# zyt334/AdaFace

Measured on AMD Instinct MI355X. Metric: 512x512 images/sec @ 50 DDIM steps, batch 8, higher is better.
Workload: dtype bf16

## Files before the change

### adaface_amd/csrc/af_conv_gemm.hip

```cpp
#include "af_kernels.h"

#include <cstdlib>
#include <cstring>
#include <mutex>
#include <type_traits>

template <int BM, int BN> struct TileCfg {
  static constexpr int XR = BM / 32, WR = BN / 32;
  static constexpr int WM = BM / 2, WN = BN / 2;
  static constexpr int MI = WM / 32, NI = WN / 32;
  static constexpr int TILE_BYTES = (BM + BN) * 128;
  static constexpr int EPI_LD = BN + 4;
  static constexpr int EPI_BYTES = BM * EPI_LD * 4;
  static constexpr int LDS_BYTES = (2 * TILE_BYTES > EPI_BYTES) ? 2 * TILE_BYTES : EPI_BYTES;
};

__device__ __forceinline__ void lds_dma16(__amdgpu_buffer_rsrc_t rs, char* lds_base, unsigned voffset, unsigned soffset) {
#if defined(__HIP_DEVICE_COMPILE__)
  __builtin_amdgcn_raw_ptr_buffer_load_lds(rs, (__attribute__((address_space(3))) void*)lds_base, 16, voffset, soffset,
                                           0, 0);
#endif
}

__device__ __forceinline__ void tile_coords(int wg, int nwg, int ntm, int ntn, int gm, int& tm, int& tn) {
// ... 867 lines not shown
    char* base = smem + slot_off;
    pp_static_for<0, NPMAX>([&](auto qc) { stage_piece(qc, base, sc); });
    kw = kw_next(kw);
  };

  const unsigned lds0 = (unsigned)(__UINTPTR_TYPE__)((__attribute__((address_space(3))) char*)smem);
  const unsigned fch0 = (unsigned)((lane >> 4) ^ (lane & 7)) * 16u;
  const unsigned fch1 = (unsigned)(((lane >> 4) + 4) ^ (lane & 7)) * 16u;
  const unsigned x_base = (unsigned)((wq * 64 + (lane & 15)) * 128);
  const unsigned w_base = (unsigned)(XBYTES + (g * C::HN + (lane & 15)) * 128);

  f32x4 acc[NI][MI];
#pragma unroll
  for (int i = 0; i < NI; ++i)
#pragma unroll
    for (int j = 0; j < MI; ++j) acc[i][j] = f32x4{0.f, 0.f, 0.f, 0.f};
  pp_u32x4 xf[MI][2], wf[NI][2];
#pragma unroll
  for (int i = 0; i < NI; ++i) wf[i][1] = pp_u32x4{0u, 0u, 0u, 0u};
#pragma unroll
  for (int j = 0; j < MI; ++j) xf[j][1] = pp_u32x4{0u, 0u, 0u, 0u};

  auto half = [&](int slot_off, auto rc, auto mc) {
    constexpr int ur = decltype(rc)::value, um = decltype(mc)::value;
    const unsigned b = lds0 + (unsigned)slot_off + (ur ? fch1 : fch0);
    pp_static_for<0, NI * MI>([&](auto nc) {
      constexpr int n = decltype(nc)::value;
      constexpr int i = n / MI, j = n % MI;
      if constexpr (n < NI) wf[n][ur] = pp_lds_read128<n * 2048>(b + w_base);
      else if constexpr (n < NI + MI) xf[n - NI][ur] = pp_lds_read128<(n - NI) * 2048>(b + x_base);
      acc[i][j] = __builtin_amdgcn_mfma_f32_16x16x32_bf16(__builtin_bit_cast(bf16x8, wf[i][um]),
                                                          __builtin_bit_cast(bf16x8, xf[j][um]), acc[i][j], 0, 0, 0);
      if constexpr (n < NI + MI) __builtin_amdgcn_sched_barrier(0);
    });
  };
  std::integral_constant<int, 0> U0;
  std::integral_constant<int, 1> U1;

  const int cl = 4 * (lane >> 4);
  float4 bias_r[NI];
  auto load_bias = [&]() {
#pragma unroll
    for (int i = 0; i < NI; ++i) {
      bias_r[i] = float4{0.f, 0.f, 0.f, 0.f};
      if (p.bias && p.splitk <= 1) bias_r[i] = *reinterpret_cast<const float4*>(p.bias + n0 + g * C::HN + i * 16 + cl);
    }
  };
  if constexpr (!MG) load_bias();

  float4 ln_cs[LNMODE == 1 ? NI : 1];
  float ln_mu[LNMODE == 1 ? MI : 1], ln_rs[LNMODE == 1 ? MI : 1];
  if constexpr (LNMODE == 1) {
#pragma unroll
    for (int i = 0; i < NI; ++i) ln_cs[i] = *reinterpret_cast<const float4*>(p.ln_colsum + n0 + g * C::HN + i * 16 + cl);
#pragma unroll
    for (int j = 0; j < MI; ++j) {
      const int m = m0 + wq * 64 + j * 16 + (lane & 15);
      float2 st = float2{0.f, 0.f};
      if (m < p.M) st = *reinterpret_cast<const float2*>(p.ln_stats + (long)m * 2);
      ln_mu[j] = st.x;
      ln_rs[j] = st.y;
    }
  }

  pp_u32x4 w8[MG ? NI : 1][2], xa8[MG ? MI : 1][2], xb8[MG ? MI : 1][2];
  int wsc8[FP8 ? NI : 1];
  int xsc8 = p.x_scale_e8;
  if constexpr (MG && !FP8) {
#pragma unroll
    for (int i = 0; i < NI; ++i) w8[i][0] = w8[i][1] = pp_u32x4{0u, 0u, 0u, 0u};
#pragma unroll
    for (int j = 0; j < MI; ++j) xa8[j][0] = xa8[j][1] = xb8[j][0] = xb8[j][1] = pp_u32x4{0u, 0u, 0u, 0u};
  }
  if constexpr (FP8) {
    asm volatile("" : "+v"(xsc8));
#pragma unroll
    for (int i = 0; i < NI; ++i) {
      w8[i][0] = w8[i][1] = pp_u32x4{0u, 0u, 0u, 0u};
      wsc8[i] = (int)p.w_scale[n0 + g * C::HN + i * 16 + (lane & 15)];
    }
#pragma unroll
    for (int j = 0; j < MI; ++j) xa8[j][0] = xa8[j][1] = xb8[j][0] = xb8[j][1] = pp_u32x4{0u, 0u, 0u, 0u};
  }
  auto mfma8 = [&](f32x4& c, const pp_u32x4 (&wv)[2], const pp_u32x4 (&xv)[2], int wscale) {
    if constexpr (!FP8) {
      c = __builtin_amdgcn_mfma_f32_16x16x32_bf16(__builtin_bit_cast(bf16x8, wv[0]), __builtin_bit_cast(bf16x8, xv[0]), c, 0, 0, 0);
      c = __builtin_amdgcn_mfma_f32_16x16x32_bf16(__builtin_bit_cast(bf16x8, wv[1]), __builtin_bit_cast(bf16x8, xv[1]), c, 0, 0, 0);
      asm volatile("" : "+v"(c));
      return;
    }
    const pp_i32x8 a = __builtin_shufflevector(__builtin_bit_cast(pp_i32x4, wv[0]), __builtin_bit_cast(pp_i32x4, wv[1]), 0, 1, 2, 3, 4, 5, 6, 7);
    const pp_i32x8 b = __builtin_shufflevector(__builtin_bit_cast(pp_i32x4, xv[0]), __builtin_bit_cast(pp_i32x4, xv[1]), 0, 1, 2, 3, 4, 5, 6, 7);
    c = __builtin_amdgcn_mfma_scale_f32_16x16x128_f8f6f4(a, b, c, 0, 0, 0, wscale, 0, xsc8);
    asm volatile("" : "+v"(c));
  };
  auto wait_block = [&](auto nc, pp_u32x4 (&blk)[2]) {
    constexpr int n = decltype(nc)::value;
    asm volatile("s_waitcnt lgkmcnt(%2)" : "+v"(blk[0]), "+v"(blk[1]) : "n"(n) : "memory");
  };
#ifdef AF_LAB_ABLATE
  const int lab = p.ablate >> 4;
#else
  constexpr int lab = 0;
#endif
  auto cphase8 = [&](int slot_off, pp_u32x4 (&xc)[MG ? MI : 1][2], pp_u32x4 (&xp)[MG ? MI : 1][2], int stage_off,
                     const StageCtx& sc) {
    if constexpr (MG) {
      constexpr int NB = NI + MI;
      char* sbase = smem + stage_off;
      const unsigned b0 = lds0 + (unsigned)slot_off + fch0, b1 = lds0 + (unsigned)slot_off + fch1;
      auto rd_block = [&](auto bc) {
        constexpr int bi = decltype(bc)::value;
        if (lab & 2) return;
        if constexpr (bi == 0) {
          w8[0][0] = pp_lds_read128<0>(b0 + w_base);
          w8[0][1] = pp_lds_read128<0>(b1 + w_base);
        } else if constexpr (bi <= MI) {
          xc[bi - 1][0] = pp_lds_read128<(bi - 1) * 2048>(b0 + x_base);
          xc[bi - 1][1] = pp_lds_read128<(bi - 1) * 2048>(b1 + x_base);
        } else {
          w8[bi - MI][0] = pp_lds_read128<(bi - MI) * 2048>(b0 + w_base);
          w8[bi - MI][1] = pp_lds_read128<(bi - MI) * 2048>(b1 + w_base);
        }
      };
      rd_block(std::integral_constant<int, 0>{});
      rd_block(std::integral_constant<int, 1>{});
      __builtin_amdgcn_sched_barrier(0);
      pp_static_for<0, MI * NI>([&](auto mc) {
        constexpr int m = decltype(mc)::value;
        if constexpr (m < MI) {
          if (!(lab & 4)) mfma8(acc[NI - 1][m], w8[NI - 1], xp[m], wsc8[FP8 ? NI - 1 : 0]);
        } else {
          constexpr int i = (m - MI) / MI, j = (m - MI) % MI;
          constexpr int issued = (2 + m) < NB ? (2 + m) : NB;
          constexpr int need = i == 0 ? 1 + j : (j == 0 ? MI + i : -1);
          if constexpr (need >= 0) {
            std::integral_constant<int, 2 * (issued - need - 1)> cnt;
            if constexpr (i == 0) wait_block(cnt, xc[j]); else wait_block(cnt, w8[i]);
            if constexpr (i == 0 && j == 0) wait_block(cnt, w8[0]);
          }
          if (!(lab & 4)) mfma8(acc[i][j], w8[i], xc[j], wsc8[FP8 ? i : 0]);
        }
        if constexpr (2 + m < NB) rd_block(std::integral_constant<int, 2 + m>{});
        if constexpr (m >= MI && (m - MI) / 2 < NPMAX) {
          if (!(lab & 1) && g == ((m - MI) & 1)) stage_piece(std::integral_constant<int, (m - MI) / 2>{}, sbase, sc);
        }
        __builtin_amdgcn_sched_barrier(0);
      });
      static_assert(MI + 2 * (NPMAX - 1) + 1 < MI * NI, "merged schedule: a staging slot behind an MFMA for every piece");
      pp_wait_lgkm0();
    }
  };

  int rd = 0, w0 = SLOT, w1 = 2 * SLOT;
  if constexpr (MG) {
    stage(0);
    stage(SLOT);
    auto tile = [&](auto& xc, auto& xp) {
      if (g == 0) pp_wait_vm<NP0>(); else pp_wait_vm<NP1>();
      __builtin_amdgcn_s_barrier();
      const StageCtx sc = stage_begin(kw);
      cphase8(rd, xc, xp, w1, sc);
      kw = kw_next(kw);
      const int tmp = rd; rd = w0; w0 = w1; w1 = tmp;
    };
    for (int t = 0; t + 1 < KT; t += 2) {
      tile(xa8, xb8);
      tile(xb8, xa8);
    }
    if (KT & 1) tile(xa8, xb8);
    pp_wait_vm<0>();
    if (KT & 1) {
#pragma unroll
      for (int j = 0; j < MI; ++j) mfma8(acc[NI - 1][j], w8[NI - 1], xa8[j], wsc8[FP8 ? NI - 1 : 0]);
    } else {
#pragma unroll
      for (int j = 0; j < MI; ++j) mfma8(acc[NI - 1][j], w8[NI - 1], xb8[j], wsc8[FP8 ? NI - 1 : 0]);
    }
    __builtin_amdgcn_s_barrier();
  } else {
    auto wait_keep1 = [&]() { if (g == 0) pp_wait_vm<NP0>(); else pp_wait_vm<NP1>(); };
    stage(0);
    if (g == 1) {
      if (KT > 1) { stage(SLOT); wait_keep1(); } else pp_wait_vm<0>();
    }
    __builtin_amdgcn_s_barrier();
    if (g == 1) __builtin_amdgcn_s_barrier();
    auto dphase = [&](int t) {
      if (g == 0) {
        if (t + 1 < KT) { stage(w0); wait_keep1(); } else pp_wait_vm<0>();
      } else {
        if (t + 2 < KT) stage(w1);
      }
      __builtin_amdgcn_s_barrier();
    };
    auto cend = [&](int t) {
      if (g == 1) { if (t + 2 < KT) wait_keep1(); else pp_wait_vm<0>(); }
      __builtin_amdgcn_s_barrier();
      const int tmp = rd; rd = w0; w0 = w1; w1 = tmp;
    };
    for (int t = 0; t < KT; ++t) {
      dphase(t);
      __builtin_amdgcn_s_setprio(1);
      half(rd, U0, U1);
      pp_wait_lgkm0();
      half(rd, U1, U0);
      pp_wait_lgkm0();
      __builtin_amdgcn_s_setprio(0);
      cend(t);
    }
#pragma unroll
    for (int i = 0; i < NI; ++i)
#pragma unroll
      for (int j = 0; j < MI; ++j)
        acc[i][j] = __builtin_amdgcn_mfma_f32_16x16x32_bf16(__builtin_bit_cast(bf16x8, wf[i][1]),
                                                            __builtin_bit_cast(bf16x8, xf[j][1]), acc[i][j], 0, 0, 0);
    if (g == 0) __builtin_amdgcn_s_barrier();
  }
  if constexpr (MG) load_bias();

  pp_epilogue<BN, LNMODE>(p, acc, bias_r, ln_cs, ln_mu, ln_rs, smem, tid, lane, g, wq, m0, n0, tn, zk);
}

#ifdef AF_LAB_ABLATE
__device__ unsigned long long g_lab_stamps[2048 * 5];
extern "C" int af_lab_stamps(unsigned long long* out, int n) {
  return hipMemcpyFromSymbol(out, HIP_SYMBOL(g_lab_stamps), sizeof(unsigned long long) * (size_t)n) == hipSuccess ? 0 : -1;
}
__device__ __forceinline__ unsigned long long lab_now() {
  unsigned long long t;
  __builtin_amdgcn_sched_barrier(0);
  asm volatile("s_memrealtime %0\n\ts_waitcnt lgkmcnt(0)" : "=s"(t)::"memory");
  __builtin_amdgcn_sched_barrier(0);
  return t;
}
#endif
struct Halo8Cfg {
  static constexpr int BN = 160;
  static constexpr int HPIX = 400, HBUF = HPIX * 128, WBYTES = BN * 128;
  static constexpr int W_BASE = 2 * HBUF, LDS_BYTES = 2 * HBUF + 3 * WBYTES;
  static constexpr int NHQ = 7;
  static_assert(LDS_BYTES <= 160 * 1024, "LDS budget");
};

template <int LABL>
__global__ __launch_bounds__(512) void conv3x3_halo8_kernel(const ConvGemmParams p) {
  using C = PpCfg<160>;
  using H = Halo8Cfg;
  typedef bf16 T;
  constexpr int BN = 160, NI = C::NI, MI = C::MI, NHQ = H::NHQ;
  extern __shared__ __attribute__((aligned(1024))) char smem[];
  const int tid = threadIdx.x, lane = tid & 63, wid = __builtin_amdgcn_readfirstlane(tid >> 6);
  const int g = wid >> 2, wq = wid & 3;
  const int ntm = p.M / 256, ntn = p.N / BN;
  int tm, tn;
  tile_coords(blockIdx.x, gridDim.x, ntm, ntn, p.group_m, tm, tn);
  const int m0 = tm * 256, n0 = tn * BN;
  const int zk = blockIdx.z;
  T* const xsrc = const_cast<T*>(reinterpret_cast<const T*>(p.src));
  T* const wsrc = const_cast<T*>(reinterpret_cast<const T*>(p.W));
  const __amdgpu_buffer_rsrc_t rs_x = __builtin_amdgcn_make_buffer_rsrc(xsrc, 0, (int)0xFFFFFFF0u, 0x00020000);
  const __amdgpu_buffer_rsrc_t rs_w = __builtin_amdgcn_make_buffer_rsrc(wsrc, 0, (int)0xFFFFFFF0u, 0x00020000);

  const int KT_all = p.K / 64;
  const int kt_per = (KT_all + p.splitk - 1) / p.splitk;
  const int kt_begin = zk * kt_per;
#ifdef AF_LAB_ABLATE
  const int lab = p.ablate >> 4;
  const int KT = (lab & 16) ? 9 : min(KT_all, kt_begin + kt_per) - kt_begin;
#else
  constexpr int lab = 0;
  const int KT = min(KT_all, kt_begin + kt_per) - kt_begin;
#endif
  const int chunk0 = kt_begin / 9;
  const int nch = KT / 9;
#ifdef AF_LAB_ABLATE
  unsigned long long st0 = 0, st1 = 0, st2 = 0;
  if (lab & 64) st0 = lab_now();
#endif

  const int Wo = p.Wo, HW = Wo + 2, wsh = p.wo_shift;
  const int R = 256 >> wsh;
  const int HP = (R + 2) * HW;
  const int img = m0 >> p.howo_shift;
  const int y0 = (m0 & (p.Ho * Wo - 1)) >> wsh;
  const int srow = lane >> 3;
  const unsigned dchunk = (unsigned)((lane & 7) ^ srow);
  const unsigned ldcb = (unsigned)p.ldc * 2u;

  unsigned h_off[NHQ];
  const int nhq = (H::HPIX / 8 - 1 - wid) / 8 + 1;
#pragma unroll
  for (int q = 0; q < NHQ; ++q) {
    const int hp = (wid + 8 * q) * 8 + srow;
    const int hy = hp / HW, hx = hp - hy * HW;
    const int iy = y0 - 1 + hy, ix = hx - 1;
    const bool ok = hp < HP && (unsigned)iy < (unsigned)p.Hi && (unsigned)ix < (unsigned)p.Wi;
    h_off[q] = ok ? (unsigned)((long)img * p.src_batch_stride * 2) + (unsigned)((iy >> p.up) * p.Ws + (ix >> p.up)) * ldcb + dchunk * 16u
                  : 0xFFFFFFFFu;
  }
  const unsigned hl6 = (unsigned)(wid < 2 ? 8 * (NHQ - 1) * 1024 : 0);
  if (wid >= 2) h_off[NHQ - 1] = h_off[0];
  unsigned w_off[3];
#pragma unroll
  for (int q = 0; q < 3; ++q) {
    const int n = n0 + (wid + 8 * q) * 8 + srow;
    w_off[q] = (n < p.Wrows && (wid + 8 * q) < BN / 8) ? (unsigned)((long)n * p.ldw * 2) + dchunk * 16u : 0xFFFFFFFFu;
  }
// ... 1714 lines not shown
```

### adaface_amd/csrc/af_conv_s8.hip

```cpp
#include "af_kernels.h"

#include <type_traits>

namespace cs8 {
typedef bf16 T;
typedef __attribute__((ext_vector_type(4))) unsigned u32x4;
constexpr int BM = 256, BN = 80, NI = 5, MI = 2, SPLITK = 4;
constexpr int HSLOTS = 448, HBUF = HSLOTS * 128, NHQ = HSLOTS / 8 / 8;
constexpr int WBYTES = BN * 128, WPIECES = BN / 8, D = 3, NS = 4;
constexpr int W_BASE = 2 * HBUF, LDS_BYTES = W_BASE + NS * WBYTES;
static_assert(LDS_BYTES <= 160 * 1024 && NHQ == 7, "LDS plan");

__device__ __forceinline__ void lds_dma16(__amdgpu_buffer_rsrc_t rs, char* lds_base, unsigned voffset, unsigned soffset) {
#if defined(__HIP_DEVICE_COMPILE__)
  __builtin_amdgcn_raw_ptr_buffer_load_lds(rs, (__attribute__((address_space(3))) void*)lds_base, 16, voffset, soffset, 0, 0);
#endif
}
__device__ __forceinline__ u32x4 lds_read128(unsigned addr) {
  u32x4 v;
  asm volatile("ds_read_b128 %0, %1" : "=v"(v) : "v"(addr) : "memory");
  return v;
}
template <int OFF> __device__ __forceinline__ u32x4 lds_read128o(unsigned addr) {
  u32x4 v;
  asm volatile("ds_read_b128 %0, %1 offset:%2" : "=v"(v) : "v"(addr), "n"(OFF) : "memory");
  return v;
}
template <int N> __device__ __forceinline__ void wait_vm() { asm volatile("s_waitcnt vmcnt(%0)" ::"n"(N) : "memory"); }
template <int N> __device__ __forceinline__ void wait_lgkm2(u32x4& a, u32x4& b) {
  asm volatile("s_waitcnt lgkmcnt(%2)" : "+v"(a), "+v"(b) : "n"(N) : "memory");
}
template <int N> __device__ __forceinline__ void wait_lgkm4(u32x4& a, u32x4& b, u32x4& c, u32x4& d) {
  asm volatile("s_waitcnt lgkmcnt(%4)" : "+v"(a), "+v"(b), "+v"(c), "+v"(d) : "n"(N) : "memory");
}
template <int I, int N, typename F> __device__ __forceinline__ void static_for(F&& f) {
  if constexpr (I < N) {
    f(std::integral_constant<int, I>{});
    static_for<I + 1, N>(f);
  }
}
__device__ __forceinline__ f32x4 mma(const u32x4& a, const u32x4& b, const f32x4& c) {
  return __builtin_amdgcn_mfma_f32_16x16x32_bf16(__builtin_bit_cast(bf16x8, a), __builtin_bit_cast(bf16x8, b), c, 0, 0, 0);
}

template <int SPLITK_T>
__global__ __launch_bounds__(512) void conv3x3_s8_kernel(const ConvGemmParams p) {
  extern __shared__ __attribute__((aligned(1024))) char smem[];
  const int tid = threadIdx.x, lane = tid & 63, wid = __builtin_amdgcn_readfirstlane(tid >> 6);
  const int l15 = lane & 15, g = lane >> 4;
  const int ntn = p.N / BN;
  const int tm = blockIdx.x / ntn, tn = blockIdx.x - tm * ntn;
  const int m0 = tm * BM, n0 = tn * BN, zk = blockIdx.z;
  const int nch = (p.Cin >> 6) / SPLITK_T, chunk0 = zk * nch;
  const __amdgpu_buffer_rsrc_t rs_x = __builtin_amdgcn_make_buffer_rsrc(const_cast<T*>(reinterpret_cast<const T*>(p.src)), 0, (int)0xFFFFFFF0u, 0x00020000);
  const __amdgpu_buffer_rsrc_t rs_w = __builtin_amdgcn_make_buffer_rsrc(const_cast<T*>(reinterpret_cast<const T*>(p.W)), 0, (int)0xFFFFFFF0u, 0x00020000);

  const int srow = lane >> 3;
  const unsigned dchunk = (unsigned)((lane & 7) ^ srow);
  const unsigned ldcb = (unsigned)p.ldc * 2u;
  const int wsh = p.wo_shift, Wo = 1 << wsh, HW = Wo + 2, hwsh = p.howo_shift;
  const int R = min(p.Ho, 256 >> wsh), HP1 = (R + 2) * HW, ipt = 256 / (R << wsh);
  const int img0 = m0 >> hwsh, y0 = (m0 & ((1 << hwsh) - 1)) >> wsh;
  unsigned h_off[NHQ];
#pragma unroll
  for (int q = 0; q < NHQ; ++q) {
    const int hp = (wid + 8 * q) * 8 + srow;
    const int img = hp / HP1, rem = hp - img * HP1, hy = rem / HW, hx = rem - hy * HW;
    const int iy = y0 + hy - 1, ix = hx - 1;
    const bool ok = img < ipt && (unsigned)iy < (unsigned)p.Ho && (unsigned)ix < (unsigned)Wo;
    h_off[q] = ok ? (unsigned)(((img0 + img) << hwsh) + (iy << wsh) + ix) * ldcb + dchunk * 16u : 0xFFFFFFFFu;
  }
  const int nwq = wid < WPIECES - 8 ? 2 : 1;
  unsigned w_off[2];
#pragma unroll
  for (int q = 0; q < 2; ++q) w_off[q] = (unsigned)((n0 + (wid + 8 * q) * 8 + srow) * p.ldw * 2) + dchunk * 16u;

  const int nsteps = nch * 9;
  auto stage_w = [&](int s, int slot) {
    const int c = s / 9, tap = s - 9 * c;
    const bool live = s < nsteps;
    const unsigned k0b = (unsigned)(tap * p.Cin + (chunk0 + c) * 64) * 2u;
    lds_dma16(rs_w, smem + W_BASE + slot * WBYTES + wid * 1024, live ? w_off[0] : 0xFFFFFFFFu, k0b);
    if (wid < WPIECES - 8) lds_dma16(rs_w, smem + W_BASE + slot * WBYTES + (wid + 8) * 1024, live ? w_off[1] : 0xFFFFFFFFu, k0b);
  };
  auto stage_h = [&](auto qc, int hbuf, int c) {
    constexpr int q = decltype(qc)::value;
    const bool live = c < nch;
    lds_dma16(rs_x, smem + hbuf * HBUF + (wid + 8 * q) * 1024, live ? h_off[q] : 0xFFFFFFFFu, (unsigned)(chunk0 + c) * 128u);
  };

  const unsigned lds0 = (unsigned)(__UINTPTR_TYPE__)((__attribute__((address_space(3))) char*)smem);
  const unsigned fch0 = (unsigned)(g ^ (lane & 7)) * 16u, fch1 = (unsigned)((g + 4) ^ (lane & 7)) * 16u;
  const unsigned w_base = (unsigned)(l15 * 128);
  int xhp[MI];
#pragma unroll
  for (int j = 0; j < MI; ++j) {
    const int t = wid * 32 + j * 16 + l15;
    const int part = t / (R << wsh), yl = (t >> wsh) - part * R;
    xhp[j] = part * HP1 + yl * HW + (t & (Wo - 1));
  }
  f32x4 acc[NI][MI];
#pragma unroll
  for (int i = 0; i < NI; ++i)
#pragma unroll
    for (int j = 0; j < MI; ++j) acc[i][j] = f32x4{0.f, 0.f, 0.f, 0.f};

  static_for<0, NHQ>([&](auto qc) { stage_h(qc, 0, 0); });
#pragma unroll
  for (int s = 0; s < D; ++s) stage_w(s, s);

  u32x4 xs[2][MI][2], wh[2][2][2];
#pragma unroll
  for (int j = 0; j < MI; ++j) xs[1][j][0] = xs[1][j][1] = u32x4{0u, 0u, 0u, 0u};
#pragma unroll
  for (int b2 = 0; b2 < 2; ++b2) wh[1][b2][0] = wh[1][b2][1] = u32x4{0u, 0u, 0u, 0u};
  int hb = 0, slot = 0;
  for (int c = 0; c < nch; ++c) {
    static_for<0, 9>([&](auto tc) {
      constexpr int tap = decltype(tc)::value;
      constexpr int cs = tap & 1, ps = cs ^ 1;
      constexpr int hyoung = tap == 0 ? 0 : (tap == 1 ? 1 : (tap == 2 ? 2 : (tap <= 7 ? 3 : 2)));
      if (nwq == 2) wait_vm<2 * (D - 1) + hyoung>(); else wait_vm<(D - 1) + hyoung>();
      __builtin_amdgcn_s_barrier();
      constexpr int ky = tap / 3, kx = tap - 3 * ky;
      const int tapoff = ky * HW + kx;
      unsigned xa[MI];
#pragma unroll
      for (int j = 0; j < MI; ++j) {
        const unsigned hp = (unsigned)(xhp[j] + tapoff);
        xa[j] = lds0 + (unsigned)(hb * HBUF) + (hp << 7) + ((((unsigned)g ^ hp) & 7u) << 4);
      }
      const unsigned wa0 = lds0 + (unsigned)(W_BASE + slot * WBYTES) + w_base + fch0;
      const unsigned wa1 = lds0 + (unsigned)(W_BASE + slot * WBYTES) + w_base + fch1;
      u32x4 wf[3][2];
#pragma unroll
      for (int j = 0; j < MI; ++j) {
        xs[cs][j][0] = lds_read128(xa[j]);
        xs[cs][j][1] = lds_read128(xa[j] ^ 64u);
      }
      wf[0][0] = lds_read128o<0 * 2048>(wa0); wf[0][1] = lds_read128o<0 * 2048>(wa1);
      wf[1][0] = lds_read128o<1 * 2048>(wa0); wf[1][1] = lds_read128o<1 * 2048>(wa1);
      wf[2][0] = lds_read128o<2 * 2048>(wa0); wf[2][1] = lds_read128o<2 * 2048>(wa1);
      __builtin_amdgcn_sched_barrier(0);
#pragma unroll
      for (int b2 = 0; b2 < 2; ++b2)
#pragma unroll
        for (int j = 0; j < MI; ++j) {
          acc[3 + b2][j] = mma(wh[ps][b2][0], xs[ps][j][0], acc[3 + b2][j]);
          acc[3 + b2][j] = mma(wh[ps][b2][1], xs[ps][j][1], acc[3 + b2][j]);
          asm volatile("" : "+v"(acc[3 + b2][j]));
        }
      __builtin_amdgcn_sched_barrier(0);
      wait_lgkm4<4>(xs[cs][0][0], xs[cs][0][1], xs[cs][1][0], xs[cs][1][1]);
      wait_lgkm2<4>(wf[0][0], wf[0][1]);
#pragma unroll
      for (int j = 0; j < MI; ++j) {
        acc[0][j] = mma(wf[0][0], xs[cs][j][0], acc[0][j]);
        acc[0][j] = mma(wf[0][1], xs[cs][j][1], acc[0][j]);
        asm volatile("" : "+v"(acc[0][j]));
      }
      wh[cs][0][0] = lds_read128o<3 * 2048>(wa0); wh[cs][0][1] = lds_read128o<3 * 2048>(wa1);
      __builtin_amdgcn_sched_barrier(0);
      wait_lgkm2<4>(wf[1][0], wf[1][1]);
#pragma unroll
      for (int j = 0; j < MI; ++j) {
        acc[1][j] = mma(wf[1][0], xs[cs][j][0], acc[1][j]);
        acc[1][j] = mma(wf[1][1], xs[cs][j][1], acc[1][j]);
        asm volatile("" : "+v"(acc[1][j]));
      }
      stage_w(c * 9 + tap + D, (slot + D) & (NS - 1));
      if constexpr (tap < NHQ) stage_h(std::integral_constant<int, tap>{}, hb ^ 1, c + 1);
      wh[cs][1][0] = lds_read128o<4 * 2048>(wa0); wh[cs][1][1] = lds_read128o<4 * 2048>(wa1);
      __builtin_amdgcn_sched_barrier(0);
      wait_lgkm2<4>(wf[2][0], wf[2][1]);
#pragma unroll
      for (int j = 0; j < MI; ++j) {
        acc[2][j] = mma(wf[2][0], xs[cs][j][0], acc[2][j]);
        acc[2][j] = mma(wf[2][1], xs[cs][j][1], acc[2][j]);
        asm volatile("" : "+v"(acc[2][j]));
      }
      __builtin_amdgcn_sched_barrier(0);
      asm volatile("s_waitcnt lgkmcnt(0)"
                   : "+v"(wh[cs][0][0]), "+v"(wh[cs][0][1]), "+v"(wh[cs][1][0]), "+v"(wh[cs][1][1])
                   :
                   : "memory");
      slot = (slot + 1) & (NS - 1);
    });
#pragma unroll
    for (int j = 0; j < MI; ++j) { xs[1][j][0] = xs[0][j][0]; xs[1][j][1] = xs[0][j][1]; }
#pragma unroll
    for (int b2 = 0; b2 < 2; ++b2) { wh[1][b2][0] = wh[0][b2][0]; wh[1][b2][1] = wh[0][b2][1]; }
    hb ^= 1;
  }
#pragma unroll
  for (int b2 = 0; b2 < 2; ++b2)
#pragma unroll
    for (int j = 0; j < MI; ++j) {
      acc[3 + b2][j] = mma(wh[1][b2][0], xs[1][j][0], acc[3 + b2][j]);
      acc[3 + b2][j] = mma(wh[1][b2][1], xs[1][j][1], acc[3 + b2][j]);
    }
  wait_vm<0>();

  if constexpr (SPLITK_T > 1) {
    float* slab = reinterpret_cast<float*>(p.ws) + (long)zk * p.M * p.N;
#pragma unroll
    for (int j = 0; j < MI; ++j) {
      const int m = m0 + wid * 32 + j * 16 + l15;
#pragma unroll
      for (int i = 0; i < NI; ++i) *reinterpret_cast<f32x4*>(slab + (long)m * p.N + n0 + i * 16 + 4 * g) = acc[i][j];
    }
  } else {
    __builtin_amdgcn_s_barrier();
    constexpr int OPITCH = BN * 2 + 16, OCH = BN / 8, NST = 32 * OCH / 64;
    char* otile = smem + wid * (32 * OPITCH);
    const T* res = reinterpret_cast<const T*>(p.residual);
    const T* rowb = reinterpret_cast<const T*>(p.rowbias);
    const int cl = 4 * g;
    float4 bvec[NI];
    Quad<T> bq[NI];
#pragma unroll
    for (int i = 0; i < NI; ++i) {
      bvec[i] = p.bias ? *reinterpret_cast<const float4*>(p.bias + n0 + i * 16 + cl) : float4{0.f, 0.f, 0.f, 0.f};
      if (rowb) bq[i].load(rowb + (long)(m0 >> p.howo_shift) * p.ldrb + n0 + i * 16 + cl);
    }
#pragma unroll
    for (int j = 0; j < MI; ++j) {
      const int m = m0 + wid * 32 + j * 16 + l15;
      Quad<T> rq[NI];
      if (res) {
#pragma unroll
        for (int i = 0; i < NI; ++i) rq[i].load(res + (long)m * p.ldr + n0 + i * 16 + cl);
      }
#pragma unroll
      for (int i = 0; i < NI; ++i) {
        const float* bp = reinterpret_cast<const float*>(&bvec[i]);
        Quad<T> o;
#pragma unroll
        for (int e = 0; e < 4; ++e) {
          float v = acc[i][j][e] + bp[e];
          if (rowb) v += to_f32<T>(bq[i].e[e]);
          if (res) v += to_f32<T>(rq[i].e[e]);
          o.e[e] = from_f32<T>(v);
        }
        o.store(reinterpret_cast<T*>(otile + (j * 16 + l15) * OPITCH) + i * 16 + cl);
      }
    }
    const __amdgpu_buffer_rsrc_t rs_o = __builtin_amdgcn_make_buffer_rsrc(reinterpret_cast<T*>(p.out), 0, (int)0xFFFFFFF0u, 0x00020000);
    u32x4 chunk[NST];
    unsigned orow[NST];
#pragma unroll
    for (int i = 0; i < NST; ++i) {
      const unsigned c = (unsigned)(lane + 64 * i), row = c / OCH, ch = c - row * OCH;
      orow[i] = (unsigned)(m0 + wid * 32 + (int)row) * (unsigned)(p.ldo * 2) + ch * 16u;
      chunk[i] = *reinterpret_cast<const u32x4*>(otile + row * OPITCH + ch * 16);
    }
    __builtin_amdgcn_sched_barrier(0);
#pragma unroll
    for (int i = 0; i < NST; ++i) __builtin_amdgcn_raw_buffer_store_b128(chunk[i], rs_o, orow[i], n0 * 2, 0);
    __builtin_amdgcn_sched_barrier(0);
  }
}
}

int af_conv_s8_slices(const ConvGemmParams& p, int batch) {
  auto pow2 = [](int v) { return v > 0 && (v & (v - 1)) == 0; };
  if (batch != 1 || p.fp8 || p.ks != 3 || p.stride != 1 || p.pad != 1 || p.up != 0 || p.Hi != p.Ho || p.Wi != p.Wo ||
      p.Hs != p.Ho || p.Ws != p.Wo || !pow2(p.Wo) || !pow2(p.Ho) || p.Wo < 8 || p.Wo > 64 || p.M <= 0 || p.M % cs8::BM != 0 || p.N % cs8::BN != 0 ||
      p.K != 9 * p.Cin || p.ldc < p.Cin || p.ldc % 8 != 0 || p.epilogue != AF_EPI_NONE || p.ln_stats || p.ln_stats_out || p.gn_ab || p.phase4 ||
      p.src_batch_stride != (long)p.Ho * p.Wo * p.ldc)
    return 0;
  const int R = p.Ho < 256 / p.Wo ? p.Ho : 256 / p.Wo;
  if (256 % (R * p.Wo) != 0 || (256 / (R * p.Wo)) * (R + 2) * (p.Wo + 2) > cs8::HSLOTS || (p.Ho * p.Wo > 256 && p.Ho % R != 0)) return 0;
  if (p.Wo == 8 && p.Ho == 8) return p.Cin % (64 * cs8::SPLITK) == 0 ? cs8::SPLITK : 0;
  return (p.Cin % 64 == 0 && p.ldo % 8 == 0 && (!p.residual || p.ldr % 4 == 0) && (!p.rowbias || p.ldrb % 4 == 0) && ((__UINTPTR_TYPE__)p.out & 15) == 0 &&
          (long)(p.M / cs8::BM) * (p.N / cs8::BN) >= 128) ? 1 : 0;
}
bool af_conv_s8_ok(const ConvGemmParams& p, int batch) { return af_conv_s8_slices(p, batch) != 0; }
int af_launch_conv_s8(const ConvGemmParams& p, hipStream_t stream) {
  static unsigned long long attr_done4 = 0, attr_done1 = 0;
  const int sl = af_conv_s8_slices(p, 1);
  if (sl == 0 || p.splitk != sl || (sl > 1 && !p.ws) || p.wo_shift < 3 || p.howo_shift < p.wo_shift) {
    af_set_error_msg("conv_s8: shape / slice count %d not taken by the small-map kernel", p.splitk);
    return -1;
  }
  const dim3 grid((p.M / cs8::BM) * (p.N / cs8::BN), 1, sl);
  if (sl > 1) {
    if (int rc = af_ensure_dynamic_lds(attr_done4, reinterpret_cast<const void*>(&cs8::conv3x3_s8_kernel<cs8::SPLITK>), cs8::LDS_BYTES)) return rc;
    hipLaunchKernelGGL(cs8::conv3x3_s8_kernel<cs8::SPLITK>, grid, dim3(512), cs8::LDS_BYTES, stream, p);
  } else {
    if (int rc = af_ensure_dynamic_lds(attr_done1, reinterpret_cast<const void*>(&cs8::conv3x3_s8_kernel<1>), cs8::LDS_BYTES)) return rc;
    hipLaunchKernelGGL(cs8::conv3x3_s8_kernel<1>, grid, dim3(512), cs8::LDS_BYTES, stream, p);
  }
  HIP_CHECK_RET(hipGetLastError());
  return 0;
}
```

Before: 10.99.

## Specialize bf16 merged-group GEMM main loop with compile-time slot rotation and incremental walk

Adds a dedicated main-loop path for the non-FP8 merged-group case. The loop is unrolled six steps deep so the triple-buffer LDS slot offsets and register ping-pong choices become compile-time constants. The runtime index swaps and per-tile stage_begin/kw_next recomputation are replaced by an incremental walk struct that carries channel, tap and offset state forward. The group branch (g) is hoisted out of the loop. This should cut scalar address arithmetic and branching per K-tile, at the cost of larger code size and more register pressure.

```diff
diff --git a/adaface_amd/csrc/af_conv_gemm.hip b/adaface_amd/csrc/af_conv_gemm.hip
--- a/adaface_amd/csrc/af_conv_gemm.hip
+++ b/adaface_amd/csrc/af_conv_gemm.hip
@@ -1043,8 +1043,176 @@
     }
   };
 
+  struct PpWalk {
+    int kt, tap, kx;
+    unsigned c0b, k0b;
+    unsigned delta;
+  };
+  struct PpStage {
+    __amdgpu_buffer_rsrc_t rx, rw;
+    unsigned c0b, k0b, delta;
+    int tapbit;
+  };
+  const int kt_end = kt_begin + KT;
+  const unsigned cin2 = (unsigned)p.Cin * 2u, rowstep = (unsigned)(p.Ws - p.ks + 1) * ldcb;
+  auto walk_next = [&](PpWalk w) -> PpWalk {
+    ++w.kt;
+    if constexpr (GATHER) {
+      const bool row = w.kx + 1 == p.ks, chunk = w.tap + 1 == taps8;
+      w.kx = row ? 0 : w.kx + 1;
+      w.delta = chunk ? 0u : w.delta + (row ? rowstep : ldcb);
+      w.c0b += chunk ? 128u : 0u;
+      w.k0b = chunk ? w.c0b : w.k0b + cin2;
+      w.tap = chunk ? 0 : w.tap + 1;
+    } else {
+      w.c0b += 128u;
+      w.k0b = w.c0b;
+    }
+    return w;
+  };
+  auto stage_vals = [&](const PpWalk& w) -> PpStage {
+    PpStage s;
+    const int nrec = w.kt < kt_end ? (int)0xFFFFFFF0u : 0;
+    s.rx = __builtin_amdgcn_make_buffer_rsrc(const_cast<T*>(reinterpret_cast<const T*>(p.src)), 0, nrec, 0x00020000);
+    s.rw = __builtin_amdgcn_make_buffer_rsrc(const_cast<T*>(reinterpret_cast<const T*>(p.W)), 0, nrec, 0x00020000);
+    s.c0b = w.c0b;
+    s.k0b = w.k0b;
+    s.delta = w.delta;
+    s.tapbit = 1 << w.tap;
+#ifdef AF_LAB_ABLATE
+    if ((p.ablate & 0x100) && w.tap) s.tapbit = 0;
+#endif
+    return s;
+  };
+  auto piece16 = [&](auto qc, auto gc, char* base, const PpStage& s) {
+    constexpr int q = decltype(qc)::value, G = decltype(gc)::value;
+    constexpr int NX = G ? NX1 : NX0, NP = G ? NP1 : NP0, XB = G ? XP0 : 0, WB = G ? WP0 : 0;
+    if constexpr (q < NX) {
+      unsigned a = x_off[q];
+      if constexpr (GATHER) a = (x_yx[q] & s.tapbit) ? a + s.delta : 0xFFFFFFFFu;
+      lds_dma16(s.rx, base + (XB + wq + 4 * q) * 1024, a, s.c0b);
+    } else if constexpr (q < NP) {
+      lds_dma16(s.rw, base + XBYTES + (WB + wq + 4 * (q - NX)) * 1024, w_off[q - NX], s.k0b);
+    }
+  };
+  auto step16 = [&](auto sc, auto gc, PpWalk w) -> PpWalk {
+    constexpr int S = decltype(sc)::value, G = decltype(gc)::value;
+    constexpr int NB = NI + MI, RD = (S % 3) * SLOT, ST = ((S + 2) % 3) * SLOT;
+    auto& xc = (S & 1) ? xb8 : xa8;
+    auto& xp = (S & 1) ? xa8 : xb8;
+    pp_wait_vm<G ? NP1 : NP0>();
+    __builtin_amdgcn_s_barrier();
+    const PpStage s = stage_vals(w);
+    const unsigned b0 = lds0 + (unsigned)RD + fch0, b1 = lds0 + (unsigned)RD + fch1;
+    auto rd_block = [&](auto bc) {
+      constexpr int bi = decltype(bc)::value;
+      if (lab & 2) return;
+      if constexpr (bi == 0) {
+        w8[0][0] = pp_lds_read128<0>(b0 + w_base);
+        w8[0][1] = pp_lds_read128<0>(b1 + w_base);
+      } else if constexpr (bi <= MI) {
+        xc[bi - 1][0] = pp_lds_read128<(bi - 1) * 2048>(b0 + x_base);
+        xc[bi - 1][1] = pp_lds_read128<(bi - 1) * 2048>(b1 + x_base);
+      } else {
+        w8[bi - MI][0] = pp_lds_read128<(bi - MI) * 2048>(b0 + w_base);
+        w8[bi - MI][1] = pp_lds_read128<(bi - MI) * 2048>(b1 + w_base);
+      }
+    };
+    rd_block(std::integral_constant<int, 0>{});
+    rd_block(std::integral_constant<int, 1>{});
+    __builtin_amdgcn_sched_barrier(0);
+    pp_static_for<0, MI * NI>([&](auto mc) {
+      constexpr int m = decltype(mc)::value;
+      if constexpr (m < MI) {
+        if (!(lab & 4)) mfma8(acc[NI - 1][m], w8[NI - 1], xp[m], 0);
+      } else {
+        constexpr int i = (m - MI) / MI, j = (m - MI) % MI;
+        constexpr int issued = (2 + m) < NB ? (2 + m) : NB;
+        constexpr int need = i == 0 ? 1 + j : (j == 0 ? MI + i : -1);
+        if constexpr (need >= 0) {
+          std::integral_constant<int, 2 * (issued - need - 1)> cnt;
+          if constexpr (i == 0) wait_block(cnt, xc[j]); else wait_block(cnt, w8[i]);
+          if constexpr (i == 0 && j == 0) wait_block(cnt, w8[0]);
+        }
+        if (!(lab & 4)) mfma8(acc[i][j], w8[i], xc[j], 0);
+      }
+      if constexpr (2 + m < NB) rd_block(std::integral_constant<int, 2 + m>{});
+      if constexpr (m >= MI && ((m - MI) & 1) == G && (m - MI) / 2 < NPMAX) {
+        if (!(lab & 1)) piece16(std::integral_constant<int, (m - MI) / 2>{}, gc, smem + ST, s);
+      }
+      __builtin_amdgcn_sched_barrier(0);
+    });
+    pp_wait_lgkm0();
+    return walk_next(w);
+  };
+  auto run16 = [&](auto gc, PpWalk w) {
+    std::integral_constant<int, 0> S0; std::integral_constant<int, 1> S1; std::integral_constant<int, 2> S2;
+    std::integral_constant<int, 3> S3; std::integral_constant<int, 4> S4; std::integral_constant<int, 5> S5;
+    for (int n = KT / 6; n > 0; --n) {
+      w = step16(S0, gc, w);
+      w = step16(S1, gc, w);
+      w = step16(S2, gc, w);
+      w = step16(S3, gc, w);
+      w = step16(S4, gc, w);
+      w = step16(S5, gc, w);
+    }
+    const int r = KT % 6;
+    if (r > 0) {
+      w = step16(S0, gc, w);
+      if (r > 1) {
+        w = step16(S1, gc, w);
+        if (r > 2) {
+          w = step16(S2, gc, w);
+          if (r > 3) {
+            w = step16(S3, gc, w);
+            if (r > 4) step16(S4, gc, w);
+          }
+        }
+      }
+    }
+  };
+
   int rd = 0, w0 = SLOT, w1 = 2 * SLOT;
-  if constexpr (MG) {
+  if constexpr (MG && !FP8) {
+    PpWalk w;
+    {
+      const int cc = kt_begin / taps8, tap = kt_begin - cc * taps8, ky = tap / p.ks;
+      w.kt = kt_begin;
+      w.tap = tap;
+      w.kx = tap - ky * p.ks;
+      w.c0b = (unsigned)cc * 128u;
+      w.k0b = (unsigned)(tap * p.Cin + cc * 64) * 2u;
+      w.delta = (unsigned)(ky * p.Ws + w.kx) * ldcb;
+    }
+    std::integral_constant<int, 0> G0;
+    std::integral_constant<int, 1> G1;
+    auto stage16 = [&](auto gc, auto slc, const PpWalk& k) {
+      const PpStage s = stage_vals(k);
+      pp_static_for<0, NPMAX>([&](auto qc) { piece16(qc, gc, smem + decltype(slc)::value * SLOT, s); });
+    };
+    std::integral_constant<int, 0> L0;
+    std::integral_constant<int, 1> L1;
+    if (g == 0) {
+      stage16(G0, L0, w);
+      w = walk_next(w);
+      stage16(G0, L1, w);
+      run16(G0, walk_next(w));
+    } else {
+      stage16(G1, L0, w);
+      w = walk_next(w);
+      stage16(G1, L1, w);
+      run16(G1, walk_next(w));
+    }
+    pp_wait_vm<0>();
+    if (KT & 1) {
+#pragma unroll
+      for (int j = 0; j < MI; ++j) mfma8(acc[NI - 1][j], w8[NI - 1], xa8[j], 0);
+    } else {
+#pragma unroll
+      for (int j = 0; j < MI; ++j) mfma8(acc[NI - 1][j], w8[NI - 1], xb8[j], 0);
+    }
+    __builtin_amdgcn_s_barrier();
+  } else if constexpr (MG) {
     stage(0);
     stage(SLOT);
     auto tile = [&](auto& xc, auto& xp) {
```

Result: no change. 11.02 (median of 6 runs) (+0.3%).

## Restage small-map conv pipeline per kernel row with interleaved LDS prefetch

Applied to the files above, without the earlier changes.

Reworks the 3x3 small-map conv main loop so weights are staged one kernel row (three taps) at a time into two double-buffered slots, and the halo buffer shrinks to 50 pieces. LDS reads for the next tap are interleaved with the MFMA blocks of the current tap, with fine-grained lgkmcnt waits. Global-memory waits and barriers now happen only once per kernel row instead of every tap. It also adds compile-time ablation variants behind AF_LAB_ABLATE that can skip DMA, LDS reads or MFMAs for lab experiments. The risk is the hand-tuned waitcnt counts: if any is wrong the kernel reads stale data, and the extra in-flight reads can raise register pressure.

```diff
diff --git a/adaface_amd/csrc/af_conv_s8.hip b/adaface_amd/csrc/af_conv_s8.hip
--- a/adaface_amd/csrc/af_conv_s8.hip
+++ b/adaface_amd/csrc/af_conv_s8.hip
@@ -6,24 +6,20 @@
 typedef bf16 T;
 typedef __attribute__((ext_vector_type(4))) unsigned u32x4;
 constexpr int BM = 256, BN = 80, NI = 5, MI = 2, SPLITK = 4;
-constexpr int HSLOTS = 448, HBUF = HSLOTS * 128, NHQ = HSLOTS / 8 / 8;
-constexpr int WBYTES = BN * 128, WPIECES = BN / 8, D = 3, NS = 4;
-constexpr int W_BASE = 2 * HBUF, LDS_BYTES = W_BASE + NS * WBYTES;
-static_assert(LDS_BYTES <= 160 * 1024 && NHQ == 7, "LDS plan");
+constexpr int HPIECES = 50, HSLOTS = HPIECES * 8, HBUF = HSLOTS * 128, NHQ = 7;
+constexpr int WBYTES = BN * 128, WPIECES = BN / 8, WSLOT = 3 * WBYTES;
+constexpr int W_BASE = 2 * HBUF, LDS_BYTES = W_BASE + 2 * WSLOT;
+static_assert(LDS_BYTES <= 160 * 1024 && (NHQ - 1) * 8 < HPIECES && NHQ * 8 >= HPIECES && HPIECES - 48 == WPIECES - 8, "LDS plan");
 
 __device__ __forceinline__ void lds_dma16(__amdgpu_buffer_rsrc_t rs, char* lds_base, unsigned voffset, unsigned soffset) {
 #if defined(__HIP_DEVICE_COMPILE__)
   __builtin_amdgcn_raw_ptr_buffer_load_lds(rs, (__attribute__((address_space(3))) void*)lds_base, 16, voffset, soffset, 0, 0);
 #endif
 }
-__device__ __forceinline__ u32x4 lds_read128(unsigned addr) {
+template <int LABL, int OFF> __device__ __forceinline__ u32x4 lds_read128o(unsigned addr) {
   u32x4 v;
-  asm volatile("ds_read_b128 %0, %1" : "=v"(v) : "v"(addr) : "memory");
-  return v;
-}
-template <int OFF> __device__ __forceinline__ u32x4 lds_read128o(unsigned addr) {
-  u32x4 v;
-  asm volatile("ds_read_b128 %0, %1 offset:%2" : "=v"(v) : "v"(addr), "n"(OFF) : "memory");
+  if constexpr ((LABL & 2) != 0) asm volatile("" : "=v"(v) : "v"(addr) : "memory");
+  else asm volatile("ds_read_b128 %0, %1 offset:%2" : "=v"(v) : "v"(addr), "n"(OFF) : "memory");
   return v;
 }
 template <int N> __device__ __forceinline__ void wait_vm() { asm volatile("s_waitcnt vmcnt(%0)" ::"n"(N) : "memory"); }
@@ -39,12 +35,17 @@
     static_for<I + 1, N>(f);
   }
 }
-__device__ __forceinline__ f32x4 mma(const u32x4& a, const u32x4& b, const f32x4& c) {
-  return __builtin_amdgcn_mfma_f32_16x16x32_bf16(__builtin_bit_cast(bf16x8, a), __builtin_bit_cast(bf16x8, b), c, 0, 0, 0);
-}
-
-template <int SPLITK_T>
-__global__ __launch_bounds__(512) void conv3x3_s8_kernel(const ConvGemmParams p) {
+template <int LABL> __device__ __forceinline__ f32x4 mma(const u32x4& a, const u32x4& b, const f32x4& c) {
+  if constexpr ((LABL & 4) != 0) {
+    f32x4 d = c;
+    asm volatile("" : "+v"(d) : "v"(a), "v"(b));
+    return d;
+  } else {
+    return __builtin_amdgcn_mfma_f32_16x16x32_bf16(__builtin_bit_cast(bf16x8, a), __builtin_bit_cast(bf16x8, b), c, 0, 0, 0);
+  }
+}
+
+template <int SPLITK_T, int LABL> __device__ __forceinline__ void conv3x3_s8_body(const ConvGemmParams& p) {
   extern __shared__ __attribute__((aligned(1024))) char smem[];
   const int tid = threadIdx.x, lane = tid & 63, wid = __builtin_amdgcn_readfirstlane(tid >> 6);
   const int l15 = lane & 15, g = lane >> 4;
@@ -70,18 +71,23 @@
     const bool ok = img < ipt && (unsigned)iy < (unsigned)p.Ho && (unsigned)ix < (unsigned)Wo;
     h_off[q] = ok ? (unsigned)(((img0 + img) << hwsh) + (iy << wsh) + ix) * ldcb + dchunk * 16u : 0xFFFFFFFFu;
   }
-  const int nwq = wid < WPIECES - 8 ? 2 : 1;
+  const bool two = wid < WPIECES - 8;
   unsigned w_off[2];
 #pragma unroll
   for (int q = 0; q < 2; ++q) w_off[q] = (unsigned)((n0 + (wid + 8 * q) * 8 + srow) * p.ldw * 2) + dchunk * 16u;
 
-  const int nsteps = nch * 9;
-  auto stage_w = [&](int s, int slot) {
-    const int c = s / 9, tap = s - 9 * c;
-    const bool live = s < nsteps;
-    const unsigned k0b = (unsigned)(tap * p.Cin + (chunk0 + c) * 64) * 2u;
-    lds_dma16(rs_w, smem + W_BASE + slot * WBYTES + wid * 1024, live ? w_off[0] : 0xFFFFFFFFu, k0b);
-    if (wid < WPIECES - 8) lds_dma16(rs_w, smem + W_BASE + slot * WBYTES + (wid + 8) * 1024, live ? w_off[1] : 0xFFFFFFFFu, k0b);
+  auto stage_w = [&](auto kxc, auto qc, int c, int ky, int slot) {
+    constexpr int kx = decltype(kxc)::value, q = decltype(qc)::value;
+    const bool live = c < nch;
+    const unsigned k0b = (unsigned)((3 * ky + kx) * p.Cin + (chunk0 + c) * 64) * 2u;
+    lds_dma16(rs_w, smem + W_BASE + slot * WSLOT + kx * WBYTES + (wid + 8 * q) * 1024, live ? w_off[q] : 0xFFFFFFFFu, k0b);
+  };
+  auto stage_step_w = [&](auto kxc, int c, int ky, int slot) {
+    constexpr int kx = decltype(kxc)::value;
+    stage_w(kxc, std::integral_constant<int, 0>{}, c, ky, slot);
+    if constexpr (kx == 2) {
+      if (two) static_for<0, 3>([&](auto k2) { stage_w(k2, std::integral_constant<int, 1>{}, c, ky, slot); });
+    }
   };
   auto stage_h = [&](auto qc, int hbuf, int c) {
     constexpr int q = decltype(qc)::value;
@@ -105,99 +111,100 @@
 #pragma unroll
     for (int j = 0; j < MI; ++j) acc[i][j] = f32x4{0.f, 0.f, 0.f, 0.f};
 
-  static_for<0, NHQ>([&](auto qc) { stage_h(qc, 0, 0); });
-#pragma unroll
-  for (int s = 0; s < D; ++s) stage_w(s, s);
-
-  u32x4 xs[2][MI][2], wh[2][2][2];
+  static_for<0, NHQ - 1>([&](auto qc) { stage_h(qc, 0, 0); });
+  if (two) stage_h(std::integral_constant<int, NHQ - 1>{}, 0, 0);
+  static_for<0, 3>([&](auto kxc) { stage_step_w(kxc, 0, 0, 0); });
+
+  u32x4 xs[2][MI][2], wf[2][NI][2];
 #pragma unroll
   for (int j = 0; j < MI; ++j) xs[1][j][0] = xs[1][j][1] = u32x4{0u, 0u, 0u, 0u};
 #pragma unroll
-  for (int b2 = 0; b2 < 2; ++b2) wh[1][b2][0] = wh[1][b2][1] = u32x4{0u, 0u, 0u, 0u};
+  for (int b = 3; b < NI; ++b) wf[1][b][0] = wf[1][b][1] = u32x4{0u, 0u, 0u, 0u};
   int hb = 0, slot = 0;
+  if constexpr ((LABL & 8) == 0)
   for (int c = 0; c < nch; ++c) {
     static_for<0, 9>([&](auto tc) {
       constexpr int tap = decltype(tc)::value;
-      constexpr int cs = tap & 1, ps = cs ^ 1;
-      constexpr int hyoung = tap == 0 ? 0 : (tap == 1 ? 1 : (tap == 2 ? 2 : (tap <= 7 ? 3 : 2)));
-      if (nwq == 2) wait_vm<2 * (D - 1) + hyoung>(); else wait_vm<(D - 1) + hyoung>();
-      __builtin_amdgcn_s_barrier();
-      constexpr int ky = tap / 3, kx = tap - 3 * ky;
-      const int tapoff = ky * HW + kx;
-      unsigned xa[MI];
-#pragma unroll
-      for (int j = 0; j < MI; ++j) {
-        const unsigned hp = (unsigned)(xhp[j] + tapoff);
-        xa[j] = lds0 + (unsigned)(hb * HBUF) + (hp << 7) + ((((unsigned)g ^ hp) & 7u) << 4);
+      constexpr int ky = tap / 3, kx = tap - 3 * ky, cs = tap & 1, ps = cs ^ 1;
+      auto read_part = [&](auto tnc, auto stc, auto partc) {
+        constexpr int tn = decltype(tnc)::value, st = decltype(stc)::value, part = decltype(partc)::value;
+        constexpr int kyn = tn / 3, kxn = tn - 3 * kyn;
+        if constexpr (part == 0) {
+#pragma unroll
+          for (int j = 0; j < MI; ++j) {
+            const unsigned hp = (unsigned)(xhp[j] + kyn * HW + kxn);
+            const unsigned xa = lds0 + (unsigned)(hb * HBUF) + (hp << 7) + ((((unsigned)g ^ hp) & 7u) << 4);
+            xs[st][j][0] = lds_read128o<LABL, 0>(xa);
+            xs[st][j][1] = lds_read128o<LABL, 0>(xa ^ 64u);
+          }
+        } else {
+          const unsigned wa = lds0 + (unsigned)(W_BASE + slot * WSLOT) + w_base;
+          wf[st][part - 1][0] = lds_read128o<LABL, kxn * WBYTES + (part - 1) * 2048>(wa + fch0);
+          wf[st][part - 1][1] = lds_read128o<LABL, kxn * WBYTES + (part - 1) * 2048>(wa + fch1);
+        }
+      };
+      auto mma_block = [&](auto bc, auto stc) {
+        constexpr int b = decltype(bc)::value, st = decltype(stc)::value;
+#pragma unroll
+        for (int j = 0; j < MI; ++j) {
+          acc[b][j] = mma<LABL>(wf[st][b][0], xs[st][j][0], acc[b][j]);
+          acc[b][j] = mma<LABL>(wf[st][b][1], xs[st][j][1], acc[b][j]);
+          asm volatile("" : "+v"(acc[b][j]));
+        }
+      };
+      constexpr bool dma = (LABL & 1) == 0;
+      if constexpr (kx == 0) {
+        wait_vm<ky == 0 ? 0 : 2>();
+        __builtin_amdgcn_s_barrier();
+        static_for<0, 1 + NI>([&](auto partc) { read_part(tc, std::integral_constant<int, cs>{}, partc); });
+        __builtin_amdgcn_sched_barrier(0);
+        mma_block(std::integral_constant<int, 3>{}, std::integral_constant<int, ps>{});
+        mma_block(std::integral_constant<int, 4>{}, std::integral_constant<int, ps>{});
+        __builtin_amdgcn_sched_barrier(0);
       }
-      const unsigned wa0 = lds0 + (unsigned)(W_BASE + slot * WBYTES) + w_base + fch0;
-      const unsigned wa1 = lds0 + (unsigned)(W_BASE + slot * WBYTES) + w_base + fch1;
-      u32x4 wf[3][2];
-#pragma unroll
-      for (int j = 0; j < MI; ++j) {
-        xs[cs][j][0] = lds_read128(xa[j]);
-        xs[cs][j][1] = lds_read128(xa[j] ^ 64u);
+      static_for<0, NI>([&](auto bc) {
+        constexpr int b = decltype(bc)::value;
+        if constexpr (kx < 2 || b < 3) {
+          constexpr int younger = 2 * (NI - 1 - b) + (kx < 2 ? (b == 0 ? 0 : 4 + 2 * (b - 1)) : 0);
+          wait_lgkm4<younger>(xs[cs][0][0], xs[cs][0][1], xs[cs][1][0], xs[cs][1][1]);
+          wait_lgkm2<younger>(wf[cs][b][0], wf[cs][b][1]);
+          if constexpr (kx < 2) {
+            read_part(std::integral_constant<int, tap + 1>{}, std::integral_constant<int, ps>{}, std::integral_constant<int, b>{});
+            if constexpr (b == NI - 1) read_part(std::integral_constant<int, tap + 1>{}, std::integral_constant<int, ps>{}, std::integral_constant<int, NI>{});
+          }
+          __builtin_amdgcn_sched_barrier(0);
+          mma_block(bc, std::integral_constant<int, cs>{});
+          if constexpr (dma && kx == 0 && b < 3) {
+            if constexpr (ky < 2) stage_step_w(std::integral_constant<int, b>{}, c, ky + 1, slot ^ 1);
+            else stage_step_w(std::integral_constant<int, b>{}, c + 1, 0, slot ^ 1);
+          }
+          if constexpr (dma && kx == 0 && b >= 3) stage_h(std::integral_constant<int, 2 * ky + b - 3>{}, hb ^ 1, c + 1);
+          if constexpr (dma && kx == 1 && b == 0 && ky == 2) {
+            if (two) stage_h(std::integral_constant<int, NHQ - 1>{}, hb ^ 1, c + 1);
+          }
+          __builtin_amdgcn_sched_barrier(0);
+        }
+      });
+      if constexpr (kx == 2) {
+        asm volatile("s_waitcnt lgkmcnt(0)"
+                     : "+v"(wf[cs][3][0]), "+v"(wf[cs][3][1]), "+v"(wf[cs][4][0]), "+v"(wf[cs][4][1])
+                     :
+                     : "memory");
+        slot ^= 1;
       }
-      wf[0][0] = lds_read128o<0 * 2048>(wa0); wf[0][1] = lds_read128o<0 * 2048>(wa1);
-      wf[1][0] = lds_read128o<1 * 2048>(wa0); wf[1][1] = lds_read128o<1 * 2048>(wa1);
-      wf[2][0] = lds_read128o<2 * 2048>(wa0); wf[2][1] = lds_read128o<2 * 2048>(wa1);
-      __builtin_amdgcn_sched_barrier(0);
-#pragma unroll
-      for (int b2 = 0; b2 < 2; ++b2)
-#pragma unroll
-        for (int j = 0; j < MI; ++j) {
-          acc[3 + b2][j] = mma(wh[ps][b2][0], xs[ps][j][0], acc[3 + b2][j]);
-          acc[3 + b2][j] = mma(wh[ps][b2][1], xs[ps][j][1], acc[3 + b2][j]);
-          asm volatile("" : "+v"(acc[3 + b2][j]));
-        }
-      __builtin_amdgcn_sched_barrier(0);
-      wait_lgkm4<4>(xs[cs][0][0], xs[cs][0][1], xs[cs][1][0], xs[cs][1][1]);
-      wait_lgkm2<4>(wf[0][0], wf[0][1]);
-#pragma unroll
-      for (int j = 0; j < MI; ++j) {
-        acc[0][j] = mma(wf[0][0], xs[cs][j][0], acc[0][j]);
-        acc[0][j] = mma(wf[0][1], xs[cs][j][1], acc[0][j]);
-        asm volatile("" : "+v"(acc[0][j]));
-      }
-      wh[cs][0][0] = lds_read128o<3 * 2048>(wa0); wh[cs][0][1] = lds_read128o<3 * 2048>(wa1);
-      __builtin_amdgcn_sched_barrier(0);
-      wait_lgkm2<4>(wf[1][0], wf[1][1]);
-#pragma unroll
-      for (int j = 0; j < MI; ++j) {
-        acc[1][j] = mma(wf[1][0], xs[cs][j][0], acc[1][j]);
-        acc[1][j] = mma(wf[1][1], xs[cs][j][1], acc[1][j]);
-        asm volatile("" : "+v"(acc[1][j]));
-      }
-      stage_w(c * 9 + tap + D, (slot + D) & (NS - 1));
-      if constexpr (tap < NHQ) stage_h(std::integral_constant<int, tap>{}, hb ^ 1, c + 1);
-      wh[cs][1][0] = lds_read128o<4 * 2048>(wa0); wh[cs][1][1] = lds_read128o<4 * 2048>(wa1);
-      __builtin_amdgcn_sched_barrier(0);
-      wait_lgkm2<4>(wf[2][0], wf[2][1]);
-#pragma unroll
-      for (int j = 0; j < MI; ++j) {
-        acc[2][j] = mma(wf[2][0], xs[cs][j][0], acc[2][j]);
-        acc[2][j] = mma(wf[2][1], xs[cs][j][1], acc[2][j]);
-        asm volatile("" : "+v"(acc[2][j]));
-      }
-      __builtin_amdgcn_sched_barrier(0);
-      asm volatile("s_waitcnt lgkmcnt(0)"
-                   : "+v"(wh[cs][0][0]), "+v"(wh[cs][0][1]), "+v"(wh[cs][1][0]), "+v"(wh[cs][1][1])
-                   :
-                   : "memory");
-      slot = (slot + 1) & (NS - 1);
     });
 #pragma unroll
     for (int j = 0; j < MI; ++j) { xs[1][j][0] = xs[0][j][0]; xs[1][j][1] = xs[0][j][1]; }
 #pragma unroll
-    for (int b2 = 0; b2 < 2; ++b2) { wh[1][b2][0] = wh[0][b2][0]; wh[1][b2][1] = wh[0][b2][1]; }
+    for (int b = 3; b < NI; ++b) { wf[1][b][0] = wf[0][b][0]; wf[1][b][1] = wf[0][b][1]; }
     hb ^= 1;
   }
 #pragma unroll
-  for (int b2 = 0; b2 < 2; ++b2)
+  for (int b = 3; b < NI; ++b)
 #pragma unroll
     for (int j = 0; j < MI; ++j) {
-      acc[3 + b2][j] = mma(wh[1][b2][0], xs[1][j][0], acc[3 + b2][j]);
-      acc[3 + b2][j] = mma(wh[1][b2][1], xs[1][j][1], acc[3 + b2][j]);
+      acc[b][j] = mma<LABL>(wf[1][b][0], xs[1][j][0], acc[b][j]);
+      acc[b][j] = mma<LABL>(wf[1][b][1], xs[1][j][1], acc[b][j]);
     }
   wait_vm<0>();
 
@@ -260,6 +267,12 @@
     __builtin_amdgcn_sched_barrier(0);
   }
 }
+template <int SPLITK_T> __global__ __launch_bounds__(512) void conv3x3_s8_kernel(const ConvGemmParams p) { conv3x3_s8_body<SPLITK_T, 0>(p); }
+#ifdef AF_LAB_ABLATE
+template <int SPLITK_T, int LABL> __global__ __launch_bounds__(512) void conv3x3_s8_lab_kernel(const ConvGemmParams p) {
+  conv3x3_s8_body<SPLITK_T, LABL>(p);
+}
+#endif
 }
 
 int af_conv_s8_slices(const ConvGemmParams& p, int batch) {
@@ -276,21 +289,37 @@
           (long)(p.M / cs8::BM) * (p.N / cs8::BN) >= 128) ? 1 : 0;
 }
 bool af_conv_s8_ok(const ConvGemmParams& p, int batch) { return af_conv_s8_slices(p, batch) != 0; }
+template <int SL> static int launch_s8(const ConvGemmParams& p, const dim3& grid, hipStream_t stream) {
+#ifdef AF_LAB_ABLATE
+  static unsigned long long attr_lab[16] = {};
+  auto lab = [&](auto kernel, int bits) {
+    if (int rc = af_ensure_dynamic_lds(attr_lab[bits], reinterpret_cast<const void*>(kernel), cs8::LDS_BYTES)) return rc;
+    hipLaunchKernelGGL(kernel, grid, dim3(512), cs8::LDS_BYTES, stream, p);
+    HIP_CHECK_RET(hipGetLastError());
+    return 0;
+  };
+  switch ((p.ablate >> 4) & 15) {
+    case 1: return lab(&cs8::conv3x3_s8_lab_kernel<SL, 1>, 1);
+    case 2: return lab(&cs8::conv3x3_s8_lab_kernel<SL, 2>, 2);
+    case 4: return lab(&cs8::conv3x3_s8_lab_kernel<SL, 4>, 4);
+    case 6: return lab(&cs8::conv3x3_s8_lab_kernel<SL, 6>, 6);
+    case 7: return lab(&cs8::conv3x3_s8_lab_kernel<SL, 7>, 7);
+    case 8: return lab(&cs8::conv3x3_s8_lab_kernel<SL, 8>, 8);
+    default: break;
+  }
+#endif
+  static unsigned long long attr_done = 0;
+  if (int rc = af_ensure_dynamic_lds(attr_done, reinterpret_cast<const void*>(&cs8::conv3x3_s8_kernel<SL>), cs8::LDS_BYTES)) return rc;
+  hipLaunchKernelGGL(cs8::conv3x3_s8_kernel<SL>, grid, dim3(512), cs8::LDS_BYTES, stream, p);
+  HIP_CHECK_RET(hipGetLastError());
+  return 0;
+}
 int af_launch_conv_s8(const ConvGemmParams& p, hipStream_t stream) {
-  static unsigned long long attr_done4 = 0, attr_done1 = 0;
   const int sl = af_conv_s8_slices(p, 1);
   if (sl == 0 || p.splitk != sl || (sl > 1 && !p.ws) || p.wo_shift < 3 || p.howo_shift < p.wo_shift) {
     af_set_error_msg("conv_s8: shape / slice count %d not taken by the small-map kernel", p.splitk);
     return -1;
   }
   const dim3 grid((p.M / cs8::BM) * (p.N / cs8::BN), 1, sl);
-  if (sl > 1) {
-    if (int rc = af_ensure_dynamic_lds(attr_done4, reinterpret_cast<const void*>(&cs8::conv3x3_s8_kernel<cs8::SPLITK>), cs8::LDS_BYTES)) return rc;
-    hipLaunchKernelGGL(cs8::conv3x3_s8_kernel<cs8::SPLITK>, grid, dim3(512), cs8::LDS_BYTES, stream, p);
-  } else {
-    if (int rc = af_ensure_dynamic_lds(attr_done1, reinterpret_cast<const void*>(&cs8::conv3x3_s8_kernel<1>), cs8::LDS_BYTES)) return rc;
-    hipLaunchKernelGGL(cs8::conv3x3_s8_kernel<1>, grid, dim3(512), cs8::LDS_BYTES, stream, p);
-  }
-  HIP_CHECK_RET(hipGetLastError());
-  return 0;
-}
+  return sl > 1 ? launch_s8<cs8::SPLITK>(p, grid, stream) : launch_s8<1>(p, grid, stream);
+}
```

After: 10.94 before, 11.02 after (median of 6 runs). Within noise of the previous version (+0.8%).
